# hzyu17/GaussianVI

Measured on AMD Instinct MI355X. Metric: sigma-point psi-evals/sec + NGD iters/sec, 1024-factor d=12 p=5 chain, higher is better.
Workload: dtype f64; 1 GPU; c3: T=1025 states, n=6; 1 step = 1 device-resident NGD iteration; restart every 30; factor_sets_columns=[K factors, d, GH degree p, N sigma points], factor_set_kinds=1024 x quadratic-prior d=12 p=5 (N=17217); 1025 x fixed-prior d=6 p=5 (N=1433), kernel_variant=6, chunks_per_factor=4, fused_pass=True, one_launch_factor_stage=False, mirror_pairs=False, fuse_trial=2

## Files before the change

gaussianvi_amd/_lib.py:

```python
from __future__ import annotations

import ctypes as C
import os

HERE = os.path.dirname(os.path.abspath(__file__))
LIB_PATH = os.environ.get("GVI_LIB_PATH") or os.path.join(HERE, "libgvi_hip.so")

c_double_p = C.POINTER(C.c_double)
c_int32_p = C.POINTER(C.c_int32)
c_int8_p = C.POINTER(C.c_int8)
c_void_pp = C.POINTER(C.c_void_p)
ALLGATHER_FN = C.CFUNCTYPE(C.c_int, C.c_void_p, C.c_void_p, C.c_void_p, C.c_int64, C.c_void_p)

SIGNATURES = {
    "gvi_ctx_create": [C.c_int, C.c_int, c_void_pp],
    "gvi_ctx_destroy": [C.c_void_p],
    "gvi_ctx_set_stream": [C.c_void_p, C.c_void_p],
    "gvi_ctx_sync": [C.c_void_p],
    "gvi_spgh_count": [C.c_int, C.c_int, C.POINTER(C.c_int64)],
    "gvi_spgh_nodes": [C.c_int, C.c_int, C.c_int64, C.c_void_p, C.c_void_p, C.c_void_p],
    "gvi_chain_set": [C.c_void_p, C.c_int, C.c_int],
    "gvi_factors_add": [C.c_void_p, C.c_int, C.c_int, C.c_int, C.c_void_p, C.c_int, C.c_void_p, C.c_int64,
                        C.c_void_p, C.POINTER(C.c_int)],
    "gvi_factors_add_table": [C.c_void_p, C.c_int, C.c_int, C.c_int, C.c_void_p, C.c_int, C.c_void_p, C.c_int64,
                              C.c_void_p, C.c_int64, C.c_void_p, C.c_void_p, C.POINTER(C.c_int)],
    "gvi_debug_cost_log": [C.c_void_p, C.c_int, C.c_void_p, C.POINTER(C.c_double)],
    "gvi_debug_asm_launches": [C.POINTER(C.c_int64), C.POINTER(C.c_int64)],
    "gvi_debug_fused_launches": [C.POINTER(C.c_int64)],
    "gvi_debug_block3_launches": [C.POINTER(C.c_int64)],
    "gvi_debug_products": [C.c_void_p, C.c_int, C.c_void_p, C.c_void_p, C.c_void_p, C.c_void_p, C.c_void_p],
    "gvi_factors_set_table": [C.c_void_p, C.c_int, C.c_int64, C.c_void_p, C.c_void_p],
    "gvi_factors_set_sdf2d": [C.c_void_p, C.c_int, C.c_double, C.c_double, C.c_double, C.c_int, C.c_int, C.c_void_p],
    "gvi_table_file_list": [C.c_char_p, C.c_int64, C.c_void_p, C.c_void_p, C.c_void_p, C.c_void_p],
    "gvi_table_file_read": [C.c_char_p, C.c_int, C.c_int, C.c_void_p, C.c_void_p, C.c_void_p],
    "gvi_table_file_write": [C.c_char_p, C.c_int, C.c_void_p, C.c_void_p],
    "gvi_ngd_trial_publish": [C.c_void_p],
    "gvi_ngd_trial_wait": [C.c_void_p, C.c_void_p],
    "gvi_ngd_spec_gradients_local": [C.c_void_p],
    "gvi_ngd_spec_gradients_finish": [C.c_void_p],
    "gvi_ngd_accept_spec": [C.c_void_p],
    "gvi_ngd_set_update_rule": [C.c_void_p, C.c_int],
    "gvi_prox_gradients": [C.c_void_p, C.c_double],
    "gvi_prox_trial": [C.c_void_p, C.c_double, C.c_void_p],
    "gvi_prox_step": [C.c_void_p, C.c_double, C.c_int, C.c_void_p, C.c_void_p, C.c_void_p, C.c_void_p],
    "gvi_factors_set_closed_form": [C.c_void_p, C.c_int, C.c_int],
    "gvi_factors_set_sdf3d": [C.c_void_p, C.c_int, C.c_void_p, C.c_double, C.c_int, C.c_int, C.c_int, C.c_void_p],
    "gvi_factors_set_arm": [C.c_void_p, C.c_int, C.c_int, C.c_void_p, C.c_void_p, C.c_void_p, C.c_void_p, C.c_int, C.c_void_p,
                            C.c_void_p, C.c_void_p],
    "gvi_factors_set_temperature": [C.c_void_p, C.c_int, C.c_void_p],
    "gvi_factors_set_params": [C.c_void_p, C.c_int, C.c_void_p, C.c_int64],
    "gvi_factors_set_readout_rule": [C.c_void_p, C.c_int, C.c_int],
    "gvi_factors_readout_info": [C.c_void_p, C.c_int, C.POINTER(C.c_int), C.POINTER(C.c_int), C.POINTER(C.c_int),
                                 C.POINTER(C.c_int64)],
    "gvi_factors_info": [C.c_void_p, C.c_int, C.POINTER(C.c_int), C.POINTER(C.c_int), C.POINTER(C.c_int),
                         C.POINTER(C.c_int64)],
    "gvi_moments": [C.c_void_p, C.c_int] + [C.c_void_p] * 5,
    "gvi_moments_dev": [C.c_void_p, C.c_int] + [C.c_void_p] * 5,
    "gvi_raw_moments": [C.c_void_p, C.c_int] + [C.c_void_p] * 5,
    "gvi_costs": [C.c_void_p, C.c_int] + [C.c_void_p] * 3,
    "gvi_costs_dev": [C.c_void_p, C.c_int] + [C.c_void_p] * 3,
    "gvi_expand": [C.c_void_p, C.c_int] + [C.c_void_p] * 3,
    "gvi_moments_from_psi": [C.c_void_p, C.c_int] + [C.c_void_p] * 6,
    "gvi_bt_assemble": [C.c_void_p, C.c_int, C.c_void_p, C.c_void_p, C.c_void_p, C.c_void_p, C.c_void_p, C.c_void_p],
# ... 96 lines not shown
```

gaussianvi_amd/api.py:

```python
from __future__ import annotations

import ctypes as C

import numpy as np

from . import _lib

PSI_RANGE_1D, PSI_QUAD_PRIOR, PSI_FIXED_PRIOR, PSI_HOST_CALLBACK, PSI_HINGE_SDF_2D = 0, 1, 2, 3, 4
PSI_HINGE_SDF_2D_BODY, PSI_HINGE_SDF_3D, PSI_HINGE_SDF_3D_ARM = 5, 6, 7
PSI_HINGE_SDF_2D_SEG, PSI_HINGE_SDF_3D_SEG = 8, 9
PSI_HINGE_BOX = 10
PSI_HINGE_HALFSPACE = 11
PSI_HINGE_BALLS_2D, PSI_HINGE_BALLS_3D = 13, 14
RULE_NGD, RULE_PROX_JKO = 0, 1
GVI_F64, GVI_F32 = 0, 1


class GviError(RuntimeError):
    def __init__(self, status, msg):
        super().__init__(f"gvi status {status}: {msg}")
        self.status = status


def _f64(a):
# ... 554 lines not shown
    def dist_init_callback(self, rank, world, fn):
        def trampoline(user, send, recv, count, stream):
            try:
                fn(send, recv, int(count), stream)
                return 0
            except Exception:
                import traceback
                traceback.print_exc()
                return 1
        self._allgather_cb = _lib.ALLGATHER_FN(trampoline)
        self._ck(self.lib.gvi_dist_init_callback(self.h, int(rank), int(world), C.cast(self._allgather_cb, C.c_void_p), None))

    def dist_info(self):
        r, w, n = C.c_int(), C.c_int(), C.c_int()
        self._ck(self.lib.gvi_dist_info(self.h, C.byref(r), C.byref(w), C.byref(n)))
        return dict(rank=r.value, world=w.value, records_per_rank=n.value)

    def debug_cost_log(self, entries=0, read=False):
        seq = C.c_double()
        if read:
            buf = np.zeros(self._dbg_entries)
            self._ck(self.lib.gvi_debug_cost_log(self.h, 0, _p(buf), C.byref(seq)))
            return buf, seq.value
        self._dbg_entries = entries if entries > 0 else 0
        self._ck(self.lib.gvi_debug_cost_log(self.h, entries if entries > 0 else -1, None, C.byref(seq)))
        return seq.value

    def debug_products(self, sid, K, d, m):
        S, Sinv, Lam = (np.zeros((K, d, d)) for _ in range(3))
        H, u0 = np.zeros((K, d, m)), np.zeros((K, m))
        self._ck(self.lib.gvi_debug_products(self.h, sid, _p(S), _p(Sinv), _p(Lam), _p(H) if m else None, _p(u0) if m else None))
        return dict(S=S, Sinv=Sinv, Lam=Lam, H=H, u0=u0)

    def set_variant(self, v):
        self._ck(self.lib.gvi_set_variant(self.h, v))

    def set_option(self, name, value):
        self._ck(self.lib.gvi_set_option(self.h, name.encode(), int(value)))


def context_for_chain(chain, device=0, specs=None, tables=None):
    ctx = Context(device)
    ctx.chain_set(chain["T"], chain["n"])
    ids = []
    if tables:
        ctx.set_option("trust_table_degree", 1)
    for spec in (chain["specs"] if specs is None else specs):
        ids.append(ctx.factors_add(spec["d"], spec["p"], spec["start"], spec["kind"], spec["params"],
                                   spec["temperature"], table=(tables or {}).get((spec["d"], spec["p"]))))
        if spec["kind"] in (PSI_HINGE_SDF_2D, PSI_HINGE_SDF_2D_BODY, PSI_HINGE_SDF_2D_SEG):
            ctx.factors_set_sdf2d(ids[-1], spec["sdf_origin"], spec["sdf_cell"], spec["sdf_field"])
        if spec["kind"] in (PSI_HINGE_SDF_3D, PSI_HINGE_SDF_3D_ARM, PSI_HINGE_SDF_3D_SEG):
            ctx.factors_set_sdf3d(ids[-1], spec["sdf_origin"], spec["sdf_cell"], spec["sdf_field"])
        if spec["kind"] == PSI_HINGE_SDF_3D_ARM:
            ctx.factors_set_arm(ids[-1], spec["arm"])
        if spec.get("readout_order"):
            ctx.factors_set_readout_rule(ids[-1], spec["readout_order"])
    return ctx, ids
```

gaussianvi_amd/csrc/api_inspect.inc:

```

gvi_status gvi_ngd_counters(gvi_ctx* ctx, int64_t* full_passes, int64_t* cost_passes, int reset) {
  if (!ctx) return GVI_ERR_ARG;
  if (full_passes) *full_passes = ctx->ngd.n_full_pass;
  if (cost_passes) *cost_passes = ctx->ngd.n_cost_pass;
  if (reset) ctx->ngd.n_full_pass = ctx->ngd.n_cost_pass = 0;
  return GVI_OK;
}

gvi_status gvi_debug_asm_launches(int64_t* dense, int64_t* generic) {
  if (dense) *dense = chain_asm_launches()[0].load();
  if (generic) *generic = chain_asm_launches()[1].load();
  return GVI_OK;
}

gvi_status gvi_debug_fused_launches(int64_t counts[3]) {
  if (!counts) return fail(nullptr, GVI_ERR_ARG, "NULL");
  for (int i = 0; i < 3; ++i) counts[i] = fused_launches()[i].load();
  return GVI_OK;
}

gvi_status gvi_debug_block3_launches(int64_t* count) {
  if (!count) return fail(nullptr, GVI_ERR_ARG, "NULL");
  *count = block3_launches().load();
  return GVI_OK;
// ... 131 lines not shown
    HIPCK(ctx, hipMemcpyToSymbol(HIP_SYMBOL(gvi_dbg_log), &lg, sizeof(double*)));
  } else if (entries == 0 && out) {
    if (!ctx->dbg_mask) return fail(ctx, GVI_ERR_STATE, "cost log not enabled");
    HIPCK(ctx, hipMemcpy(out, ctx->dbg_log.p, (size_t)(ctx->dbg_mask + 1) * 8, hipMemcpyDeviceToHost));
  } else {
    ctx->dbg_mask = 0;
    double* lg = nullptr;
    HIPCK(ctx, hipMemcpyToSymbol(HIP_SYMBOL(gvi_dbg_log), &lg, sizeof(double*)));
  }
  if (seq_now) *seq_now = ctx->seq;
  return GVI_OK;
}

gvi_status gvi_debug_products(gvi_ctx* ctx, int set_id, double* S, double* Sinv, double* Lam, double* H, double* u0) {
  if (!ctx) return GVI_ERR_ARG;
  FactorSet* s = get_set(ctx, set_id);
  if (!s) return GVI_ERR_ARG;
  HIPCK(ctx, hipSetDevice(ctx->device));
  GVICK(sync(ctx));
  const size_t dd = (size_t)s->K * s->d * s->d * 8, md = (size_t)s->K * s->m * s->d * 8, mb = (size_t)s->K * s->m * 8;
  auto get = [&](double* out, const DevMem& src, size_t bytes) {
    if (!out || bytes == 0) return hipSuccess;
    if (!src.p || src.bytes < bytes) return hipErrorInvalidValue;
    return hipMemcpy(out, src.p, bytes, hipMemcpyDeviceToHost);
  };
  HIPCK(ctx, get(S, s->S, dd));
  HIPCK(ctx, get(Sinv, s->Sinv, dd));
  HIPCK(ctx, get(Lam, s->Lam, dd));
  HIPCK(ctx, get(H, s->H, md));
  HIPCK(ctx, get(u0, s->u0, mb));
  return GVI_OK;
}

gvi_status gvi_set_variant(gvi_ctx* ctx, int variant) {
  return ctx && route_force_of_variant(variant, &ctx->force) ? GVI_OK : GVI_ERR_ARG;
}
```

gaussianvi_amd/csrc/dpp_rowb.hpp:

```cpp
#pragma once
#include <hip/hip_runtime.h>

namespace gvi {

template <int P, int WS>
__device__ __forceinline__ double rowb_mov(const double v) {
  double o;
  if constexpr (WS > 1) asm volatile("s_nop 4\n\tv_mov_b64_dpp %0, %1 row_newbcast:%2 row_mask:0xf bank_mask:0xf" : "=v"(o) : "v"(v), "n"(P));
  else asm volatile("s_nop 1\n\tv_mov_b64_dpp %0, %1 row_newbcast:%2 row_mask:0xf bank_mask:0xf" : "=v"(o) : "v"(v), "n"(P));
  return o;
}
template <int P>
__device__ __forceinline__ void rowb_fmac(double& c, const double b) {
  asm volatile("v_fmac_f64_dpp %0, %0, %1 row_newbcast:%2 row_mask:0xf bank_mask:0xf" : "+v"(c) : "v"(b), "n"(P));
}
template <int P>
__device__ __forceinline__ void rowb_fma(double& acc, const double src, const double mul) {
  asm volatile("v_fmac_f64_dpp %0, %1, -%2 row_newbcast:%3 row_mask:0xf bank_mask:0xf" : "+v"(acc) : "v"(src), "v"(mul), "n"(P));
}
__device__ __forceinline__ void rowb_pin(double& v) { asm volatile("" : "+v"(v)); }
__device__ __forceinline__ void rowb_settle(double& v) { asm volatile("s_nop 1" : "+v"(v)); }
template <int P>
__device__ __forceinline__ int rowb_int(const int v) { return __builtin_amdgcn_update_dpp(0, v, 0x150 + P, 0xf, 0xf, false); }

}
```

gaussianvi_amd/csrc/fused_timing.inc:

```

void fused_timing_dump(gvi_ctx* c, const FusedArgs& A, const unsigned long long* stamps) {
  unsigned long long h[1120];
  (void)hipStreamSynchronize(c->stream);
  (void)hipMemcpy(h, stamps, sizeof(h), hipMemcpyDeviceToHost);
  for (int blk = 0; blk < 8; ++blk)
    for (int w = 0; w < 4; ++w)
      for (int it = 0; it < 2; ++it) {
        const unsigned long long* ws = h + 352 + ((blk * 4 + w) * 2 + it) * 12;
        fprintf(stderr, "[walk stamps] block %4d wave %d item %d: shader cycles prologue %llu | s=1 %llu (%llu tiles) | s=2 %llu (%llu) | s=3 %llu (%llu) | s=4 %llu (%llu) | reduction %llu\n",
                blk * 146, w, it, ws[0], ws[1], ws[7], ws[2], ws[8], ws[3], ws[9], ws[4], ws[10], ws[5]);
      }
  for (int w = 0; w < 4; ++w) {
    fprintf(stderr, "[prep stamps] block 0 wave %d, us after the wave's start: prologue [arguments warm | first scalars | barrier] %.2f %.2f %.2f; gather [entry | loads back | stores issued] %.2f %.2f %.2f; products [Sigma row loaded | Cholesky | L^-1 | LDS | Lam + stores | H, u0]:",
            w, (double)(long long)(h[256 + 16 * w + 11] - h[8 * w]) * 0.01, (double)(long long)(h[256 + 16 * w + 12] - h[8 * w]) * 0.01,
            (double)(long long)(h[256 + 16 * w + 13] - h[8 * w]) * 0.01, (double)(long long)(h[256 + 16 * w + 8] - h[8 * w]) * 0.01, (double)(long long)(h[256 + 16 * w + 9] - h[8 * w]) * 0.01, (double)(long long)(h[256 + 16 * w + 10] - h[8 * w]) * 0.01);
    for (int i = 0; i < 6; ++i) fprintf(stderr, " %.2f", (double)(long long)(h[256 + 16 * w + i] - h[8 * w]) * 0.01);
    fprintf(stderr, "\n");
  }
  unsigned long long t0 = ~0ull;
  for (int blk = 0; blk < 8; ++blk) if (h[blk * 32] && h[blk * 32] < t0) t0 = h[blk * 32];
  for (int blk = 0; blk < 8; ++blk)
    for (int w = 0; w < 4; ++w) {
      const unsigned hw = (unsigned)h[320 + blk * 4 + w], xcc = (unsigned)(h[320 + blk * 4 + w] >> 32);
      fprintf(stderr, "[fused stamps] block %4d wave %d (xcc %u se %u cu %2u simd %u slot %2u; absolute, us after the first start):", blk * 146, w,
// ... 11 lines not shown
    const unsigned long long* q = hb.data() + (size_t)b * 5;
    if (!q[0] || !q[2]) continue;
    const unsigned hw = (unsigned)q[3], xcc = (unsigned)(q[3] >> 32) & 15;
    auto us = [&](unsigned long long t) { return (double)(long long)(t - tb0) * 0.01; };
    cus[(xcc << 8) | ((hw >> 8) & 255)].push_back({b, us(q[0]), us(q[1]), us(q[2]), us(q[4]), hw & 15});
  }
  std::vector<double> spread_bar, spread_end, first_bar, last_bar, walk_first, walk_last;
  int shown = 0;
  for (auto& [id, v] : cus) {
    std::sort(v.begin(), v.end(), [](const Blk& a, const Blk& b) { return a.bar < b.bar; });
    double e0 = 1e300, e1 = -1e300;
    for (const Blk& x : v) { e0 = std::min(e0, x.end); e1 = std::max(e1, x.end); }
    if (v.size() == 4) {
      spread_bar.push_back(v.back().bar - v.front().bar); spread_end.push_back(e1 - e0);
      first_bar.push_back(v.front().bar); last_bar.push_back(v.back().bar);
      walk_first.push_back(v.front().bar - v.front().start); walk_last.push_back(v.back().bar - v.back().start);
    }
    if (shown++ < 6)
      for (const Blk& x : v)
        fprintf(stderr, "[cu stamps] xcc %u se %u cu %2u: block %4d slot %2u, us after the first walk start: walk start %.2f, wave 0 ends phase 2 %.2f, "
                "behind the barrier %.2f, last exit %.2f\n", id >> 8, (id >> 5) & 7, id & 31, x.b, x.slot, x.start, x.p2, x.bar, x.end);
  }
  auto stat = [](std::vector<double> v, double* med, double* mx) {
    std::sort(v.begin(), v.end());
    *med = v.empty() ? 0.0 : v[v.size() / 2]; *mx = v.empty() ? 0.0 : v.back();
  };
  double m[6], x[6];
  stat(spread_bar, &m[0], &x[0]); stat(spread_end, &m[1], &x[1]); stat(first_bar, &m[2], &x[2]); stat(last_bar, &m[3], &x[3]);
  stat(walk_first, &m[4], &x[4]); stat(walk_last, &m[5], &x[5]);
  fprintf(stderr, "[cu summary] walk_prio %d, %zu CUs with four stamped blocks (of %zu): end of phase 2 (behind the barrier), first-to-last block of a CU: "
          "median %.2f max %.2f us; first block at median %.2f, last at median %.2f max %.2f us; walk (start to barrier) of the first block median %.2f, "
          "of the last median %.2f max %.2f us; last exit, first-to-last: median %.2f max %.2f us\n", A.walk_prio, spread_bar.size(), cus.size(),
          m[0], x[0], m[2], m[3], x[3], m[4], m[5], x[5], m[1], x[1]);
}
```

gaussianvi_amd/csrc/kernels_epilogue.hpp:

```cpp
#pragma once
#include <hip/hip_runtime.h>
#include <stdint.h>

#include "device_common.hpp"
#include "factor_dev.hpp"
#include "factor_lds.hpp"

namespace gvi {

struct EpiArgs {
  FactorDev f;
  const double* partial;
  int nchunk, full;
  double* Ephi;
  double* cost;
  double* Vdmu;
  double* Vddmu;
  double* E_xmuphi;
  double* E_xxphi;
};

template <int DT>
__device__ __forceinline__ double epilogue_body_t(const EpiArgs& a, int k, double* sm, int phase, const double* P, double* Zs = nullptr) {
  const FactorDev& f = a.f;
  const int d = DT ? DT : f.d, dd = d * d, lane = threadIdx.x & 63;
  const int npo = a.full ? npairs(d) : 1;
  const EpilogueLds L{d};
  double* Ms = sm + L.Ms();
  double* M2 = Ms + (L.M2() - L.Ms());
  double* Tm = M2 + (L.Tm() - L.M2());
  double* Sv = Zs ? Zs : Tm + (L.Sv() - L.Tm());
  double* Lv = Tm + (L.Lv() - L.Tm());
  const double Tk = f.temperature[k];
  const bool want_v = a.full && (a.Vdmu || a.Vddmu);
  if (want_v && phase != 2 && !Zs) {
    const double* Sinv = f.Sinv + (size_t)k * dd;
    const double* Lam = f.Lam + (size_t)k * dd;
    for (int e = lane; e < dd; e += 64) { Sv[e] = Sinv[e]; Lv[e] = Lam[e]; }
  }
  for (int j = lane; j < npo && phase != 2; j += 64) {
    double s = 0.0;
    for (int c0 = 0; c0 < a.nchunk; c0 += 8) {
      double pv[8];
#pragma unroll
      for (int q = 0; q < 8; ++q) pv[q] = c0 + q < a.nchunk ? P[(size_t)(c0 + q) * npo + j] : 0.0;
#pragma unroll
      for (int q = 0; q < 8; ++q) s += pv[q];
    }
    Ms[j] = s;
  }
  wave_lds_sync();
  const double m0 = Ms[0];
  const double costk = m0 / Tk;
  if (lane == 0 && phase != 2) {
    if (a.Ephi) a.Ephi[k] = m0;
    if (a.cost) a.cost[k] = costk;
  }
  if (!a.full || phase == 1) return costk;
  for (int e = lane; e < dd; e += 64) {
    const int i = e / d, j = e % d;
    M2[e] = i <= j ? Ms[pair_index(d, i, j)] : Ms[pair_index(d, j, i)];
  }
  wave_lds_sync();
  if (a.Vdmu) {
    for (int i = lane; i < d; i += 64) {
      double s = 0.0;
#pragma unroll
      for (int c = 0; c < d; ++c) s += Sv[i * d + c] * Ms[1 + c];
      a.Vdmu[(size_t)k * d + i] = s / Tk;
    }
  }
  if (a.Vddmu) {
    for (int e = lane; e < dd; e += 64) {
      const int i = e / d, j = e % d;
      double s = 0.0;
#pragma unroll
      for (int c = 0; c < d; ++c) s += Sv[i * d + c] * M2[c * d + j];
      Tm[e] = s;
    }
    wave_lds_sync();
    for (int e = lane; e < dd; e += 64) {
      const int i = e / d, j = e % d;
      if (i <= j) {
        double s = 0.0;
#pragma unroll
        for (int c = 0; c < d; ++c) s += Tm[i * d + c] * Sv[j * d + c];
        double lam;
        if (Zs) {
          lam = 0.0;
#pragma unroll
          for (int c = 0; c < d; ++c) lam = fma(Sv[i * d + c], Sv[j * d + c], lam);
        } else lam = Lv[i * d + j];
        const double v = (s - lam * m0) / Tk;
        a.Vddmu[(size_t)k * dd + i * d + j] = v;
        a.Vddmu[(size_t)k * dd + j * d + i] = v;
      }
    }
    wave_lds_sync();
  }
  if (a.E_xmuphi || a.E_xxphi) {
    const double* S = f.S + (size_t)k * dd;
    for (int e = lane; e < dd; e += 64) Sv[e] = S[e];
    wave_lds_sync();
  }
  if (a.E_xmuphi) {
    for (int i = lane; i < d; i += 64) {
      double s = 0.0;
#pragma unroll
      for (int c = 0; c < d; ++c) s += Sv[i * d + c] * Ms[1 + c];
      a.E_xmuphi[(size_t)k * d + i] = s;
    }
  }
  if (a.E_xxphi) {
    for (int e = lane; e < dd; e += 64) {
      const int i = e / d, j = e % d;
      double s = 0.0;
#pragma unroll
      for (int c = 0; c < d; ++c) s += Sv[i * d + c] * M2[c * d + j];
      Tm[e] = s;
    }
    wave_lds_sync();
    for (int e = lane; e < dd; e += 64) {
      const int i = e / d, j = e % d;
      double s = 0.0;
#pragma unroll
      for (int c = 0; c < d; ++c) s += Tm[i * d + c] * Sv[j * d + c];
      a.E_xxphi[(size_t)k * dd + e] = s;
    }
  }
  return costk;
}
// ... 69 lines not shown
    acc[0] = total;
    if (host_out) {
      publish_to_host(host_out, total + half_logdet[0], seq);
    }
  }
}

constexpr int EPI_GROUP = 64;
struct EpiTail {
  int on;
  double* acc;
  const double* half_logdet;
  double* host_out;
  double seq;
  unsigned* counter;
  const double* pred;
  double pred_val;
  double* accept;
  double* cost_dev;
  int slot_cur, slot_trial;
  int c0_use_imm;
  double c0_imm;
  int safe;
};

struct CostList {
  int nsets;
  double* cost[MAX_SETS];
  int K[MAX_SETS];
};

__device__ __forceinline__ void epi_tail_arrive(const CostList& cl, const EpiTail& tail, double* cost_slot, const double costk, const int lane,
                                                const unsigned bid, const unsigned nblocks, int* last) {
  if (lane == 0) {
    __hip_atomic_store(cost_slot, costk, __ATOMIC_RELAXED, __HIP_MEMORY_SCOPE_AGENT);
    asm volatile("s_waitcnt vmcnt(0)" ::: "memory");
    const unsigned grp = bid / EPI_GROUP, ngrp = (nblocks + EPI_GROUP - 1) / EPI_GROUP;
    const unsigned in_grp = grp + 1 < ngrp ? (unsigned)EPI_GROUP : nblocks - grp * EPI_GROUP;
    unsigned* gc = tail.counter + 32u * (1u + grp);
    int l = 0;
    const bool lastg = tail.safe ? __hip_atomic_fetch_add(gc, 1u, __ATOMIC_ACQ_REL, __HIP_MEMORY_SCOPE_AGENT) == in_grp - 1
                                 : __hip_atomic_fetch_add(gc, 1u, __ATOMIC_RELAXED, __HIP_MEMORY_SCOPE_AGENT) == in_grp - 1;
    if (lastg) {
      __hip_atomic_store(gc, 0u, __ATOMIC_RELAXED, __HIP_MEMORY_SCOPE_AGENT);
      l = ngrp == 1 ? 1
                    : (tail.safe ? __hip_atomic_fetch_add(tail.counter, 1u, __ATOMIC_ACQ_REL, __HIP_MEMORY_SCOPE_AGENT) == ngrp - 1
                                 : __hip_atomic_fetch_add(tail.counter, 1u, __ATOMIC_RELAXED, __HIP_MEMORY_SCOPE_AGENT) == ngrp - 1);
    }
    *last = l;
  }
  wave_lds_sync();
  if (!*last) return;
  double total = 0.0;
  for (int s2 = 0; s2 < cl.nsets; ++s2) {
    const double* cost = cl.cost[s2];
    const int K = cl.K[s2];
    double p[4][8];
#pragma unroll
    for (int j = 0; j < 4; ++j)
#pragma unroll
      for (int q = 0; q < 8; ++q) {
        const int k = lane + 64 * j + q * 256;
        p[j][q] = k < K ? __hip_atomic_load(cost + k, __ATOMIC_RELAXED, __HIP_MEMORY_SCOPE_AGENT) : 0.0;
      }
    double vs[4];
#pragma unroll
    for (int j = 0; j < 4; ++j) {
      double s = 0.0;
#pragma unroll
      for (int q = 0; q < 8; ++q) s += p[j][q];
      for (int k0 = lane + 64 * j + 8 * 256; k0 < K; k0 += 8 * 256) {
        double pp[8];
#pragma unroll
        for (int q = 0; q < 8; ++q) {
          const int k = k0 + q * 256;
          pp[q] = k < K ? __hip_atomic_load(cost + k, __ATOMIC_RELAXED, __HIP_MEMORY_SCOPE_AGENT) : 0.0;
        }
#pragma unroll
        for (int q = 0; q < 8; ++q) s += pp[q];
      }
      vs[j] = s;
    }
    double t = (vs[0] + vs[2]) + (vs[1] + vs[3]);
#pragma unroll
    for (int w = 32; w > 0; w >>= 1) t += __shfl_down(t, w);
    total += __shfl(t, 0);
  }
  if (lane == 0) {
    __hip_atomic_store(tail.counter, 0u, __ATOMIC_RELAXED, __HIP_MEMORY_SCOPE_AGENT);
    tail.acc[0] = total;
    const double c1 = total + tail.half_logdet[0];
    if (tail.host_out) publish_to_host(tail.host_out, c1, tail.seq);
    if (tail.accept) {
      const double c0 = tail.c0_use_imm ? tail.c0_imm : tail.cost_dev[tail.slot_cur];
      tail.cost_dev[tail.slot_trial] = c1;
      tail.accept[0] = c1 < c0 ? tail.seq : 0.0;
    }
  }
  wave_lds_sync();
}

__global__ __launch_bounds__(64) void epilogue_all_kernel(EpiList L, EpiTail tail, CostList cl) {
  extern __shared__ double sm[];
  if (pred_skip(tail.pred, tail.pred_val)) return;
  int si = 0;
  while (si + 1 < L.nsets && (int)blockIdx.x >= L.koff[si + 1]) ++si;
  const int kf = (int)blockIdx.x - L.koff[si];
  if (!tail.on) { epilogue_body(L.e[si], kf, sm); return; }
  const double costk = epilogue_body(L.e[si], kf, sm, 1);
  __shared__ int last;
  epi_tail_arrive(cl, tail, L.e[si].cost + kf, costk, (int)threadIdx.x, blockIdx.x, gridDim.x, &last);
  epilogue_body(L.e[si], kf, sm, 2);
}

__global__ __launch_bounds__(256) void expand_kernel(FactorDev f, const double* __restrict__ mu,
                                                     double* __restrict__ X) {
  const int k = blockIdx.y, d = f.d;
  const int64_t i = (int64_t)blockIdx.x * 256 + threadIdx.x;
  if (i >= f.N) return;
  const double* S = f.S + (size_t)k * d * d;
  for (int r = 0; r < d; ++r) {
    double x = mu[(size_t)k * d + r];
    for (int c = 0; c < d; ++c) x += S[r * d + c] * f.Zt[(size_t)c * f.Np + i];
    X[((size_t)k * d + r) * f.N + i] = x;
  }
}

}
```

gaussianvi_amd/csrc/kernels_fused.hpp:

```cpp
#pragma once
#include "device_common.hpp"
#include "factor_lds.hpp"
#include "kernels_epilogue.hpp"
#include "kernels_orbit.hpp"
#include "kernels_prep.hpp"

namespace gvi {

constexpr int FUSED_MAX_ITEMS = 4;
constexpr int FUSED_BLOCK_STAMPS = 1100;
#ifdef GVI_FUSED_TIMING
__device__ int gvi_fused_exp;
#endif

struct FusedSet {
  FactorDev f;
  OrbitArgs oa;
  const double* mu;
  const double* Sigma;
  const int32_t* start;
  double* mu_k;
  double* Sigma_k;
  double* Ephi;
  double* cost;
  double* Vdmu;
  double* Vddmu;
};

struct FusedArgs {
  int nsets;
  int nblk;
  int koff[3];
  FusedSet s[2];
  int gather, n;
  const double* gmu;
  const double* gdmu;
// ... 39 lines not shown
    else p = A.SigU + (size_t)s * nn + c * n + (r - n);
    v[i] = e < dd ? *p : 0.0;
  }
  double m = 0.0;
  if (lane < DT) {
    const size_t j = (size_t)s * n + lane;
    m = A.gdmu ? A.gmu[j] + A.gstep * A.gdmu[j] : A.gmu[j];
  }
#ifdef GVI_FUSED_TIMING
  asm volatile("s_waitcnt vmcnt(0) lgkmcnt(0)" ::: "memory");
#endif
  PREP_STAMP(9);
  if (pred_fail(lpred)) return true;
#pragma unroll
  for (int i = 0; i < NI; ++i) {
    const int e = lane + 64 * i;
    if (e < dd) { Sl[e] = v[i]; S.Sigma_k[(size_t)k * dd + e] = v[i]; }
  }
  if (lane < DT) { ml[lane] = m; S.mu_k[(size_t)k * DT + lane] = m; }
  PREP_STAMP(10);
  return false;
}

template <int M, int SMAX, int WAVES, int D0, int D1>
__global__ __launch_bounds__(256, WAVES) void factor_fused_kernel(FusedArgs A, int dmax, int copies_max, int maxitems, [[maybe_unused]] unsigned long long* stamps) {
  extern __shared__ double sm[];
#ifdef GVI_FUSED_TIMING
#define FUSED_STAMP(i) do { const unsigned long long t_ = (i) == 0 ? t_start : __builtin_amdgcn_s_memrealtime(); if (stamps && (threadIdx.x & 63) == 0 && (blockIdx.x % 146) == 0) stamps[(blockIdx.x / 146) * 32 + (threadIdx.x >> 6) * 8 + (i)] = t_; } while (0)
  const unsigned long long t_start = __builtin_amdgcn_s_memrealtime();
#else
#define FUSED_STAMP(i) do { } while (0)
#endif
#ifdef GVI_FUSED_TIMING
  if (blockIdx.x == 0 && threadIdx.x == 0) { gvi_prep_stamps = stamps ? stamps + 8 * 32 : nullptr; gvi_walk_stamps = stamps ? stamps + 352 : nullptr; }
  unsigned long long* const bstamps = stamps && blockIdx.x < FUSED_BLOCK_STAMPS ? stamps + 1120 + blockIdx.x * 5 : nullptr;
#define FUSED_BLOCK_STAMP(i) do { if (bstamps && threadIdx.x == 0) bstamps[i] = __builtin_amdgcn_s_memrealtime(); } while (0)
  struct ExitStamp {
    unsigned long long* p;
    __device__ ~ExitStamp() { if (p && (threadIdx.x & 63) == 0) atomicMax(p, (unsigned long long)__builtin_amdgcn_s_memrealtime()); }
  } exit_stamp{bstamps ? bstamps + 4 : nullptr};
  if (bstamps && threadIdx.x == 0)
    bstamps[3] = (unsigned long long)__builtin_amdgcn_s_getreg((31 << 11) | 4) | ((unsigned long long)__builtin_amdgcn_s_getreg((31 << 11) | 20) << 32);
#else
#define FUSED_BLOCK_STAMP(i) do { } while (0)
#endif
  FUSED_STAMP(0);
#ifdef GVI_FUSED_TIMING
  if (stamps && (threadIdx.x & 63) == 0 && (blockIdx.x % 146) == 0)
    stamps[320 + (blockIdx.x / 146) * 4 + (threadIdx.x >> 6)] = (unsigned long long)__builtin_amdgcn_s_getreg((31 << 11) | 4) |
                                                                   ((unsigned long long)__builtin_amdgcn_s_getreg((31 << 11) | 20) << 32);
#endif
  const double* const pred_p = A.tail.pred;
  const int nblk_ = A.nblk, K0 = A.s[0].f.K, K1_ = A.s[1].f.K, nsets_ = A.nsets;
  constexpr int KA_LINES = (sizeof(FusedArgs) + 3 * 8 + 63) / 64;
  static_assert(KA_LINES == 28, "kernarg_warm: one specialisation per argument block size");
  kernarg_warm<KA_LINES>();
  PREP_STAMP(11);
  asm volatile("" :: "s"(pred_p), "s"(nblk_), "s"(K0), "s"(K1_), "s"(nsets_));
  PREP_STAMP(12);
  const LazyPred lpred = pred_issue(pred_p, A.tail.pred_val);
  const int wave = __builtin_amdgcn_readfirstlane(threadIdx.x >> 6);
  const int b = (int)blockIdx.x;
  if (b >= nblk_) {
    const int64_t j = (int64_t)(b - A.nblk) * 256 + threadIdx.x;
    const double v = j < A.nmu ? A.gmu[j] + A.gstep * A.gdmu[j] : 0.0;
    if (pred_fail(lpred)) return;
    if (j < A.nmu) A.mu_out[j] = v;
// ... 112 lines not shown
  FUSED_BLOCK_STAMP(1);
  __syncthreads();
  FUSED_STAMP(4);
  FUSED_BLOCK_STAMP(2);
  const bool helpers = A.tail.on && nitems <= 2;
  if (iw >= nitems) {
    const int it = iw - 2;
    if (!helpers || it < 0 || it >= nitems) return;
    const int si = it < c0 ? 0 : 1;
    const int k = b + (it < c0 ? it : it - c0) * A.nblk;
    const FusedSet& S = A.s[si];
    const double Tk = S.f.temperature[k];
    const double* Pl = Pbase + (size_t)it * ps;
    const int npo = npairs(S.f.d);
    double m0 = 0.0;
#pragma unroll
    for (int q = 0; q < 4; ++q) m0 += Pl[(size_t)q * npo];
    const double costk = m0 / Tk;
    epi_tail_arrive(A.cl, A.tail, S.cost + k, costk, (int)(threadIdx.x & 63), (unsigned)(A.koff[si] + k), (unsigned)A.koff[A.nsets],
                    (int*)(sm + (size_t)wave * region));
    return;
  }
  {
    const int si = iw < c0 ? 0 : 1;
    const int k = b + (iw < c0 ? iw : iw - c0) * A.nblk;
    const FusedSet& S = A.s[si];
    const int d = S.f.d;
    double* area = sm + (size_t)wave * region;
    double* Zs = Zbase + (size_t)iw * zs;
    const double* Pl = Pbase + (size_t)iw * ps;
    EpiArgs e;
    e.f = S.f; e.partial = nullptr; e.nchunk = 4; e.full = 1;
    e.Ephi = S.Ephi; e.cost = helpers ? nullptr : S.cost; e.Vdmu = S.Vdmu; e.Vddmu = S.Vddmu; e.E_xmuphi = nullptr; e.E_xxphi = nullptr;
    auto epi = [&](int phase) { return si == 0 ? epilogue_body_t<D0>(e, k, area, phase, Pl, Zs) : epilogue_body_t<D1>(e, k, area, phase, Pl, Zs); };
    if (!A.tail.on || helpers) { epi(0); return; }
    const double costk = epi(1);
    FUSED_STAMP(5);
    int* last = (int*)(area + EpilogueLds{d}.last());
    epi_tail_arrive(A.cl, A.tail, S.cost + k, costk, (int)(threadIdx.x & 63), (unsigned)(A.koff[si] + k), (unsigned)A.koff[A.nsets], last);
    FUSED_STAMP(6);
    epi(2);
    FUSED_STAMP(7);
  }
}

}
```

gaussianvi_amd/csrc/launch_factor.inc:

```

namespace {

template <int D, int R>
gvi_status launch_split(gvi_ctx* c, const MomArgs& a, dim3 grid, hipStream_t st) {
  const size_t lds = (size_t)SPLIT_LDS_DOUBLES(D) * 8;
  GVICK(allow_lds(c, (const void*)moments_split_kernel<D, R, true>, (int)lds));
  GVICK(allow_lds(c, (const void*)moments_split_kernel<D, R, false>, (int)lds));
  if (a.full) hipLaunchKernelGGL((moments_split_kernel<D, R, true>), grid, dim3(256), lds, st, a);
  else hipLaunchKernelGGL((moments_split_kernel<D, R, false>), grid, dim3(256), lds, st, a);
  return GVI_OK;
}

template <int D, typename Psi>
void launch_reg(const MomArgs& a, dim3 grid, hipStream_t st) {
  if (a.full) hipLaunchKernelGGL((moments_reg_kernel<D, Psi, true>), grid, dim3(256), 0, st, a);
  else hipLaunchKernelGGL((moments_reg_kernel<D, Psi, false>), grid, dim3(256), 0, st, a);
}

template <int D, int M>
void launch_sreg(const MomArgs& a, dim3 grid, hipStream_t st, bool pipe) {
  if (a.full && pipe) hipLaunchKernelGGL((moments_sreg_kernel<D, M, true, true>), grid, dim3(256), 0, st, a);
  else if (a.full) hipLaunchKernelGGL((moments_sreg_kernel<D, M, true>), grid, dim3(256), 0, st, a);
  else hipLaunchKernelGGL((moments_sreg_kernel<D, M, false>), grid, dim3(256), 0, st, a);
}
// ... 96 lines not shown

inline std::atomic<long long>& block3_launches() { static std::atomic<long long> c; return c; }

gvi_status fused_round_blocks(gvi_ctx* c, const void* kernel, size_t lds, int* out) {
  const auto key = std::make_pair(kernel, lds);
  auto it = c->fused_round.find(key);
  if (it == c->fused_round.end()) {
    int per_cu = 0, cus = 0;
    HIPCK(c, hipOccupancyMaxActiveBlocksPerMultiprocessor(&per_cu, kernel, 256, lds));
    HIPCK(c, hipDeviceGetAttribute(&cus, hipDeviceAttributeMultiprocessorCount, c->device));
    it = c->fused_round.emplace(key, per_cu * cus).first;
  }
  *out = it->second;
  return GVI_OK;
}

#ifdef GVI_FUSED_TIMING
#include "fused_timing.inc"
#endif

template <int M, int SMAX, int WAVES, int D0, int D1>
gvi_status launch_fused_t(gvi_ctx* c, FusedArgs& A, unsigned grid, size_t lds, int dmax, int copies, int items, hipEvent_t e0, hipEvent_t e1) {
  const void* const kernel = (const void*)factor_fused_kernel<M, SMAX, WAVES, D0, D1>;
  if (lds > 64 * 1024) GVICK(allow_lds(c, kernel, (int)lds));
  if (A.walk_prio) {
    int round = 0;
    GVICK(fused_round_blocks(c, kernel, lds, &round));
    if (A.nblk > round) A.walk_prio = 0;
  }
#ifdef GVI_FUSED_TIMING
  const int dbg = getenv("GVI_FUSED_DBG") ? atoi(getenv("GVI_FUSED_DBG")) : 0;
  static unsigned long long* stamps = nullptr;
  static int nprint = 0;
  constexpr size_t nstamps = 1120 + 5 * FUSED_BLOCK_STAMPS;
  if ((dbg & 8) && !stamps) {
    if (hipMalloc(&stamps, nstamps * 8) != hipSuccess) stamps = nullptr; else (void)hipMemset(stamps, 0, nstamps * 8);
    const int exp = (dbg >> 4) & 7;
    (void)hipMemcpyToSymbol(HIP_SYMBOL(gvi_fused_exp), &exp, sizeof(exp));
  }
#else
  const int dbg = 0;
  unsigned long long* stamps = nullptr;
#endif
  hipExtLaunchKernelGGL((factor_fused_kernel<M, SMAX, WAVES, D0, D1>), dim3(grid), dim3(256), (uint32_t)lds, c->stream, e0, e1, 0, A, dmax, copies, items,
                        (dbg & 8) ? stamps : (unsigned long long*)nullptr);
  ++fused_launches()[M == 2 ? 2 : (SMAX <= 4 ? 0 : 1)];
#ifdef GVI_FUSED_TIMING
  if ((dbg & 8) && stamps && ++nprint > 200 && nprint <= 202) fused_timing_dump(c, A, stamps);
#endif
  return GVI_OK;
}

gvi_status launch_prep(gvi_ctx* c, const FactorDev& f, const double* mu, const double* Sigma, hipStream_t st) {
  const size_t lds = prep_lds_bytes(f.d);
  if (!with_prep_instance(f.d, [&]<int EPLP>(PrepInst<EPLP>) { hipLaunchKernelGGL(prep_kernel<EPLP>, dim3(f.K), dim3(64), lds, st, f, mu, Sigma); }))
    return fail(c, GVI_ERR_UNSUPPORTED, "factor dimension > 32");
  return GVI_OK;
}

gvi_status run_prep(gvi_ctx* c, FactorSet& s, const double* mu, const double* Sigma, int slot = -1,
                    hipStream_t st = nullptr) {
  if (!st) st = c->stream;
  if (slot >= 0 && s.prep_slot == slot) return GVI_OK;
  s.prep_slot = slot;
  if (s.K == 0) return GVI_OK;
  GVICK(launch_prep(c, s.dev(c->opt), mu, Sigma, st));
  HIPCK(c, hipGetLastError());
// ... 293 lines not shown
```

include/gvi_hip.h:

```cpp
#ifndef GVI_HIP_H
#define GVI_HIP_H

#include <stdint.h>

#ifdef __cplusplus
extern "C" {
#endif

typedef struct gvi_ctx gvi_ctx;
typedef int gvi_status;

enum {
  GVI_OK = 0,
  GVI_ERR_ARG = 1,
  GVI_ERR_HIP = 2,
  GVI_ERR_UNSUPPORTED = 3,
  GVI_ERR_NOTABLE = 4,
  GVI_ERR_STATE = 5
};
enum { GVI_F64 = 0, GVI_F32 = 1 };

enum { GVI_PSI_RANGE_1D = 0, GVI_PSI_QUAD_PRIOR = 1, GVI_PSI_FIXED_PRIOR = 2, GVI_PSI_HOST_CALLBACK = 3,
       GVI_PSI_HINGE_SDF_2D = 4, GVI_PSI_HINGE_SDF_2D_BODY = 5, GVI_PSI_HINGE_SDF_3D = 6, GVI_PSI_HINGE_SDF_3D_ARM = 7,
       GVI_PSI_HINGE_SDF_2D_SEG = 8, GVI_PSI_HINGE_SDF_3D_SEG = 9, GVI_PSI_HINGE_BOX = 10,
// ... 115 lines not shown
gvi_status gvi_ngd_cov_columns_dev(gvi_ctx* ctx, int ncols, const int32_t* nodes, double* C_dev);

gvi_status gvi_interp_set(gvi_ctx* ctx, int Q, const int32_t* idx, const double* A, const double* B, const double* c,
                          const double* Qt);
gvi_status gvi_interp_info(gvi_ctx* ctx, int* Q, int* nbad);
gvi_status gvi_bt_interp(gvi_ctx* ctx, const double* mu, const double* SigD, const double* SigU, double* mean_q, double* cov_q);
gvi_status gvi_ngd_interp(gvi_ctx* ctx, double* mean_q, double* cov_q);
gvi_status gvi_ngd_interp_dev(gvi_ctx* ctx, double* mean_q_dev, double* cov_q_dev);
gvi_status gvi_bt_interp_samples(gvi_ctx* ctx, int S, const double* X, uint64_t noise_seed, int64_t first, const double* eps,
                                 double* Xq);
gvi_status gvi_ngd_sample_interp(gvi_ctx* ctx, int S, uint64_t seed, uint64_t noise_seed, int64_t first, double* X, double* Xq);
gvi_status gvi_ngd_sample_interp_dev(gvi_ctx* ctx, int S, uint64_t seed, uint64_t noise_seed, int64_t first, double* X_dev,
                                     double* Xq_dev);

gvi_status gvi_sample_factor_costs(gvi_ctx* ctx, int set_id, int S, const double* X, double* cost);
gvi_status gvi_sample_clearance(gvi_ctx* ctx, int set_id, int S, const double* X, double* clr);
gvi_status gvi_sample_clearance_dev(gvi_ctx* ctx, int set_id, int S, const double* X_dev, double* clr_dev);
gvi_status gvi_sample_costs(gvi_ctx* ctx, int S, const double* X, double* J);
gvi_status gvi_sample_costs_dev(gvi_ctx* ctx, int S, const double* X_dev, double* J_dev);
gvi_status gvi_ngd_sample_costs(gvi_ctx* ctx, int S, uint64_t seed, int64_t first, int clearance_set, double* X, double* J,
                                double* logq, double* clr_min);
gvi_status gvi_ngd_sample_costs_dev(gvi_ctx* ctx, int S, uint64_t seed, int64_t first, int clearance_set, double* X_dev,
                                    double* J_dev, double* logq_dev, double* clr_min_dev);

gvi_status gvi_profile_enable(gvi_ctx* ctx, int on);
gvi_status gvi_profile_last(gvi_ctx* ctx, int set_id, int what , float* ms);
gvi_status gvi_profile_stages(gvi_ctx* ctx, int on, float* mean_us, int* counts);
gvi_status gvi_profile_geometry(gvi_ctx* ctx, int set_id, int* variant, int* nchunk, int64_t* chunk);
gvi_status gvi_debug_cost_log(gvi_ctx* ctx, int entries, double* out, double* seq_now);
gvi_status gvi_debug_asm_launches(int64_t* dense, int64_t* generic);
gvi_status gvi_debug_fused_launches(int64_t counts[3]);
gvi_status gvi_debug_block3_launches(int64_t* count);
gvi_status gvi_debug_products(gvi_ctx* ctx, int set_id, double* S, double* Sinv, double* Lam, double* H, double* u0);
gvi_status gvi_set_variant(gvi_ctx* ctx, int variant);
gvi_status gvi_set_option(gvi_ctx* ctx, const char* name, int value);

#ifdef __cplusplus
}
#endif
#endif
```

Before: 235.8 billion psi-evals/s.

## Compute fused epilogue Hessian products with DPP row-broadcast FMAs in registers

Replaces the fused kernel's LDS-based epilogue, which ran the two d×d matrix products per factor through shared-memory loops with lane-strided indexing, with a register version. Each 16-lane row holds one column of M2 plus the m1 column, and the products use DPP row-broadcast FMAs. Vdmu and Vddmu are written straight from registers. The goal is to cut LDS traffic, sync points and integer index math in the per-factor tail. The old path is kept behind timing build flags, and the change also adds epilogue timing stamps and a debug readback API for factor outputs.

New measurement: 235.5 billion psi-evals/s. About the same (-0.1%).

```diff
diff --git a/gaussianvi_amd/_lib.py b/gaussianvi_amd/_lib.py
--- a/gaussianvi_amd/_lib.py
+++ b/gaussianvi_amd/_lib.py
@@ -29,6 +29,7 @@
     "gvi_debug_fused_launches": [C.POINTER(C.c_int64)],
     "gvi_debug_block3_launches": [C.POINTER(C.c_int64)],
     "gvi_debug_products": [C.c_void_p, C.c_int, C.c_void_p, C.c_void_p, C.c_void_p, C.c_void_p, C.c_void_p],
+    "gvi_debug_factor_outputs": [C.c_void_p, C.c_int, C.c_void_p, C.c_void_p, C.c_void_p, C.c_void_p],
     "gvi_factors_set_table": [C.c_void_p, C.c_int, C.c_int64, C.c_void_p, C.c_void_p],
     "gvi_factors_set_sdf2d": [C.c_void_p, C.c_int, C.c_double, C.c_double, C.c_double, C.c_int, C.c_int, C.c_void_p],
     "gvi_table_file_list": [C.c_char_p, C.c_int64, C.c_void_p, C.c_void_p, C.c_void_p, C.c_void_p],
diff --git a/gaussianvi_amd/api.py b/gaussianvi_amd/api.py
--- a/gaussianvi_amd/api.py
+++ b/gaussianvi_amd/api.py
@@ -610,6 +610,11 @@
         self._ck(self.lib.gvi_debug_products(self.h, sid, _p(S), _p(Sinv), _p(Lam), _p(H) if m else None, _p(u0) if m else None))
         return dict(S=S, Sinv=Sinv, Lam=Lam, H=H, u0=u0)
 
+    def debug_factor_outputs(self, sid, K, d):
+        Ephi, cost, Vdmu, Vddmu = np.empty(K), np.empty(K), np.empty((K, d)), np.empty((K, d, d))
+        self._ck(self.lib.gvi_debug_factor_outputs(self.h, sid, _p(Ephi), _p(cost), _p(Vdmu), _p(Vddmu)))
+        return Ephi, cost, Vdmu, Vddmu
+
     def set_variant(self, v):
         self._ck(self.lib.gvi_set_variant(self.h, v))
 
diff --git a/gaussianvi_amd/csrc/api_inspect.inc b/gaussianvi_amd/csrc/api_inspect.inc
--- a/gaussianvi_amd/csrc/api_inspect.inc
+++ b/gaussianvi_amd/csrc/api_inspect.inc
@@ -187,6 +187,25 @@
   return GVI_OK;
 }
 
+gvi_status gvi_debug_factor_outputs(gvi_ctx* ctx, int set_id, double* Ephi, double* cost, double* Vdmu, double* Vddmu) {
+  if (!ctx) return GVI_ERR_ARG;
+  FactorSet* s = get_set(ctx, set_id);
+  if (!s) return GVI_ERR_ARG;
+  HIPCK(ctx, hipSetDevice(ctx->device));
+  GVICK(sync(ctx));
+  const size_t K = (size_t)s->K, d = (size_t)s->d;
+  auto get = [&](double* out, const DevMem& src, size_t bytes) {
+    if (!out || bytes == 0) return hipSuccess;
+    if (!src.p || src.bytes < bytes) return hipErrorInvalidValue;
+    return hipMemcpy(out, src.p, bytes, hipMemcpyDeviceToHost);
+  };
+  HIPCK(ctx, get(Ephi, s->Ephi, K * 8));
+  HIPCK(ctx, get(cost, s->cost, K * 8));
+  HIPCK(ctx, get(Vdmu, s->Vdmu, K * d * 8));
+  HIPCK(ctx, get(Vddmu, s->Vddmu, K * d * d * 8));
+  return GVI_OK;
+}
+
 gvi_status gvi_set_variant(gvi_ctx* ctx, int variant) {
   return ctx && route_force_of_variant(variant, &ctx->force) ? GVI_OK : GVI_ERR_ARG;
 }
diff --git a/gaussianvi_amd/csrc/dpp_rowb.hpp b/gaussianvi_amd/csrc/dpp_rowb.hpp
--- a/gaussianvi_amd/csrc/dpp_rowb.hpp
+++ b/gaussianvi_amd/csrc/dpp_rowb.hpp
@@ -20,6 +20,7 @@
 }
 __device__ __forceinline__ void rowb_pin(double& v) { asm volatile("" : "+v"(v)); }
 __device__ __forceinline__ void rowb_settle(double& v) { asm volatile("s_nop 1" : "+v"(v)); }
+__device__ __forceinline__ void rowb_converged() { asm volatile("s_nop 4" ::: "memory"); }
 template <int P>
 __device__ __forceinline__ int rowb_int(const int v) { return __builtin_amdgcn_update_dpp(0, v, 0x150 + P, 0xf, 0xf, false); }
 
diff --git a/gaussianvi_amd/csrc/fused_timing.inc b/gaussianvi_amd/csrc/fused_timing.inc
--- a/gaussianvi_amd/csrc/fused_timing.inc
+++ b/gaussianvi_amd/csrc/fused_timing.inc
@@ -67,4 +67,26 @@
           "median %.2f max %.2f us; first block at median %.2f, last at median %.2f max %.2f us; walk (start to barrier) of the first block median %.2f, "
           "of the last median %.2f max %.2f us; last exit, first-to-last: median %.2f max %.2f us\n", A.walk_prio, spread_bar.size(), cus.size(),
           m[0], x[0], m[2], m[3], x[3], m[4], m[5], x[5], m[1], x[1]);
+  unsigned long long he[EPI_STAMP_WORDS];
+  (void)hipMemcpy(he, stamps + 1120 + 5 * (size_t)FUSED_BLOCK_STAMPS, sizeof(he), hipMemcpyDeviceToHost);
+  for (int blk = 0; blk < 8; ++blk)
+    for (int w = 0; w < 4; ++w) {
+      const unsigned long long* q = he + blk * 32 + w * 8;
+      const unsigned long long bar = hb[(size_t)blk * 146 * 5 + 2];
+      if (!q[0] || !q[4] || !bar) continue;
+      auto us = [&](unsigned long long t) { return (double)(long long)(t - bar) * 0.01; };
+      fprintf(stderr, "[epi stamps] block %4d wave %d, us behind the block's phase-2 barrier: entry %.2f | chunk sums, cost out %.2f | first product %.2f | "
+              "second product %.2f | last store issued %.2f\n", blk * 146, w, us(q[0]), us(q[1]), us(q[2]), q[3] ? us(q[3]) : -1.0, us(q[4]));
+    }
+  const unsigned long long* tl = he + 8 * 32;
+  if (tl[3]) {
+    unsigned long long end = 0;
+    for (int b = 0; b < A.nblk && b < FUSED_BLOCK_STAMPS; ++b) end = std::max(end, hb[(size_t)b * 5 + 4]);
+    const int lb = (int)tl[4];
+    const unsigned long long bar = lb < FUSED_BLOCK_STAMPS ? hb[(size_t)lb * 5 + 2] : 0;
+    auto rel = [&](unsigned long long t, unsigned long long ref) { return ref ? (double)(long long)(t - ref) * 0.01 : -1.0; };
+    fprintf(stderr, "[tail stamps] last arriver block %d, us behind its phase-2 barrier: entry %.2f | arrival counted %.2f | costs summed %.2f | published %.2f; "
+            "the publish is %.2f us after the first walk start and %.2f us before the latest exit of any block\n", lb, rel(tl[0], bar), rel(tl[1], bar),
+            rel(tl[2], bar), rel(tl[3], bar), rel(tl[3], tb0), rel(end, tl[3]));
+  }
 }
diff --git a/gaussianvi_amd/csrc/kernels_epilogue.hpp b/gaussianvi_amd/csrc/kernels_epilogue.hpp
--- a/gaussianvi_amd/csrc/kernels_epilogue.hpp
+++ b/gaussianvi_amd/csrc/kernels_epilogue.hpp
@@ -19,6 +19,32 @@
   double* E_xmuphi;
   double* E_xxphi;
 };
+
+constexpr int EPI_STAMP_WORDS = 8 * 32 + 8;
+#ifdef GVI_FUSED_TIMING
+__device__ unsigned long long* gvi_epi_stamps;
+#define EPI_STAMP(on, i) do { const unsigned long long t_ = __builtin_amdgcn_s_memrealtime(); if ((on) && (blockIdx.x % 146) == 0 && blockIdx.x / 146 < 8 && (threadIdx.x & 63) == 0 && gvi_epi_stamps) gvi_epi_stamps[(blockIdx.x / 146) * 32 + (threadIdx.x >> 6) * 8 + (i)] = t_; } while (0)
+#define EPI_TAIL_STAMP(i, v) do { if (gvi_epi_stamps) gvi_epi_stamps[8 * 32 + (i)] = (v); } while (0)
+#else
+#define EPI_STAMP(on, i) do { } while (0)
+#define EPI_TAIL_STAMP(i, v) do { } while (0)
+#endif
+
+__device__ __forceinline__ double epi_chunk_sum(const double* P, const int nchunk, const int npo, const int j) {
+  double s = 0.0;
+  for (int c0 = 0; c0 < nchunk; c0 += 8) {
+    double pv[8];
+#pragma unroll
+    for (int q = 0; q < 8; ++q) pv[q] = c0 + q < nchunk ? P[(size_t)(c0 + q) * npo + j] : 0.0;
+#pragma unroll
+    for (int q = 0; q < 8; ++q) s += pv[q];
+  }
+  return s;
+}
+__device__ __forceinline__ double epi_close_num(const double s, const double lam, const double m0) { return s - lam * m0; }
+__device__ __forceinline__ double epi_close(const double s, const double lam, const double m0, const double Tk) {
+  return epi_close_num(s, lam, m0) / Tk;
+}
 
 template <int DT>
 __device__ __forceinline__ double epilogue_body_t(const EpiArgs& a, int k, double* sm, int phase, const double* P, double* Zs = nullptr) {
@@ -38,16 +64,9 @@
     const double* Lam = f.Lam + (size_t)k * dd;
     for (int e = lane; e < dd; e += 64) { Sv[e] = Sinv[e]; Lv[e] = Lam[e]; }
   }
+  if (phase != 2) EPI_STAMP(Zs != nullptr, 0);
   for (int j = lane; j < npo && phase != 2; j += 64) {
-    double s = 0.0;
-    for (int c0 = 0; c0 < a.nchunk; c0 += 8) {
-      double pv[8];
-#pragma unroll
-      for (int q = 0; q < 8; ++q) pv[q] = c0 + q < a.nchunk ? P[(size_t)(c0 + q) * npo + j] : 0.0;
-#pragma unroll
-      for (int q = 0; q < 8; ++q) s += pv[q];
-    }
-    Ms[j] = s;
+    Ms[j] = epi_chunk_sum(P, a.nchunk, npo, j);
   }
   wave_lds_sync();
   const double m0 = Ms[0];
@@ -56,6 +75,7 @@
     if (a.Ephi) a.Ephi[k] = m0;
     if (a.cost) a.cost[k] = costk;
   }
+  if (phase != 2) EPI_STAMP(Zs != nullptr, 1);
   if (!a.full || phase == 1) return costk;
   for (int e = lane; e < dd; e += 64) {
     const int i = e / d, j = e % d;
@@ -79,6 +99,7 @@
       Tm[e] = s;
     }
     wave_lds_sync();
+    EPI_STAMP(Zs != nullptr, 2);
     for (int e = lane; e < dd; e += 64) {
       const int i = e / d, j = e % d;
       if (i <= j) {
@@ -91,12 +112,13 @@
 #pragma unroll
           for (int c = 0; c < d; ++c) lam = fma(Sv[i * d + c], Sv[j * d + c], lam);
         } else lam = Lv[i * d + j];
-        const double v = (s - lam * m0) / Tk;
+        const double v = epi_close(s, lam, m0, Tk);
         a.Vddmu[(size_t)k * dd + i * d + j] = v;
         a.Vddmu[(size_t)k * dd + j * d + i] = v;
       }
     }
     wave_lds_sync();
+    EPI_STAMP(Zs != nullptr, 4);
   }
   if (a.E_xmuphi || a.E_xxphi) {
     const double* S = f.S + (size_t)k * dd;
@@ -232,6 +254,9 @@
 
 __device__ __forceinline__ void epi_tail_arrive(const CostList& cl, const EpiTail& tail, double* cost_slot, const double costk, const int lane,
                                                 const unsigned bid, const unsigned nblocks, int* last) {
+#ifdef GVI_FUSED_TIMING
+  const unsigned long long t_entry = __builtin_amdgcn_s_memrealtime();
+#endif
   if (lane == 0) {
     __hip_atomic_store(cost_slot, costk, __ATOMIC_RELAXED, __HIP_MEMORY_SCOPE_AGENT);
     asm volatile("s_waitcnt vmcnt(0)" ::: "memory");
@@ -251,6 +276,9 @@
   }
   wave_lds_sync();
   if (!*last) return;
+#ifdef GVI_FUSED_TIMING
+  const unsigned long long t_counted = __builtin_amdgcn_s_memrealtime();
+#endif
   double total = 0.0;
   for (int s2 = 0; s2 < cl.nsets; ++s2) {
     const double* cost = cl.cost[s2];
@@ -286,6 +314,9 @@
     for (int w = 32; w > 0; w >>= 1) t += __shfl_down(t, w);
     total += __shfl(t, 0);
   }
+#ifdef GVI_FUSED_TIMING
+  const unsigned long long t_summed = __builtin_amdgcn_s_memrealtime();
+#endif
   if (lane == 0) {
     __hip_atomic_store(tail.counter, 0u, __ATOMIC_RELAXED, __HIP_MEMORY_SCOPE_AGENT);
     tail.acc[0] = total;
@@ -296,6 +327,11 @@
       tail.cost_dev[tail.slot_trial] = c1;
       tail.accept[0] = c1 < c0 ? tail.seq : 0.0;
     }
+#ifdef GVI_FUSED_TIMING
+    asm volatile("s_waitcnt vmcnt(0)" ::: "memory");
+    EPI_TAIL_STAMP(0, t_entry); EPI_TAIL_STAMP(1, t_counted); EPI_TAIL_STAMP(2, t_summed);
+    EPI_TAIL_STAMP(3, (unsigned long long)__builtin_amdgcn_s_memrealtime()); EPI_TAIL_STAMP(4, (unsigned long long)blockIdx.x);
+#endif
   }
   wave_lds_sync();
 }
diff --git a/gaussianvi_amd/csrc/kernels_epilogue_rowb.hpp b/gaussianvi_amd/csrc/kernels_epilogue_rowb.hpp
--- /dev/null
+++ b/gaussianvi_amd/csrc/kernels_epilogue_rowb.hpp
@@ -0,0 +1,99 @@
+#pragma once
+#include "dpp_rowb.hpp"
+#include "kernels_epilogue.hpp"
+
+namespace gvi {
+
+__host__ __device__ constexpr int epi_rowb_base(const int d, const int a) { return 1 + d + a * d - a * (a - 1) / 2 - a; }
+constexpr bool epi_rowb_index_ok() {
+  for (int d = 1; d <= 15; ++d)
+    for (int a = 0; a < d; ++a) {
+      if (epi_rowb_base(d, a) < 1 + a) return false;
+      for (int b = a; b < d; ++b) {
+        const int right = epi_rowb_base(d, a) + b, wrong = epi_rowb_base(d, b) + a;
+        if (right != 1 + d + a * d - a * (a - 1) / 2 + (b - a) || right > wrong) return false;
+      }
+    }
+  return true;
+}
+static_assert(epi_rowb_index_ok(), "epilogue_rowb_t: the packed index of M2[c'][c] as a minimum");
+
+template <int DT, int R, int C>
+__device__ __forceinline__ void epi_rowb_first(double (&t1)[R], double (&lam)[R], const double (&wcol)[R], const double (&nm2)[DT],
+                                               const double (&nwrow)[DT]) {
+  if constexpr (C < DT) {
+#pragma unroll
+    for (int r = 0; r < R; ++r) rowb_fma<C>(t1[r], wcol[r], nm2[C]);
+#pragma unroll
+    for (int r = 0; r < R; ++r) rowb_fma<C>(lam[r], wcol[r], nwrow[C]);
+    epi_rowb_first<DT, R, C + 1>(t1, lam, wcol, nm2, nwrow);
+  }
+}
+template <int DT, int R, int C>
+__device__ __forceinline__ void epi_rowb_second(double (&t2)[R], const double (&t1)[R], const double (&nwrow)[DT]) {
+  if constexpr (C < DT) {
+#pragma unroll
+    for (int r = 0; r < R; ++r) rowb_fma<C>(t2[r], t1[r], nwrow[C]);
+    epi_rowb_second<DT, R, C + 1>(t2, t1, nwrow);
+  }
+}
+
+template <int DT>
+__device__ __forceinline__ double epilogue_rowb_t(const EpiArgs& a, const int k, double* sm, const int phase, const double* P, const double* Zs) {
+  static_assert(DT >= 1 && DT <= 15, "one 16-lane row holds the d columns of M2 and m1 behind them");
+  constexpr int d = DT, dd = DT * DT, R = (DT + 3) / 4, npo = npairs(DT);
+  const int lane = (int)__builtin_amdgcn_mbcnt_hi(~0u, __builtin_amdgcn_mbcnt_lo(~0u, 0u)), q = lane >> 4, c = lane & 15;
+  double* Ms = sm + EpilogueLds{d}.Ms();
+  const double Tk = a.f.temperature[k];
+  if (phase != 2) EPI_STAMP(true, 0);
+  for (int j = lane; j < npo && phase != 2; j += 64) Ms[j] = epi_chunk_sum(P, a.nchunk, npo, j);
+  wave_lds_sync();
+  const double m0 = Ms[0];
+  const double costk = m0 / Tk;
+  if (lane == 0 && phase != 2) {
+    if (a.Ephi) a.Ephi[k] = m0;
+    if (a.cost) a.cost[k] = costk;
+  }
+  if (phase != 2) EPI_STAMP(true, 1);
+  if (phase == 1 || !(a.Vdmu || a.Vddmu)) return costk;
+  const int cr = c < d ? c : 0;
+  double wcol[R], nwrow[DT], nm2[DT];
+#pragma unroll
+  for (int r = 0; r < R; ++r) {
+    const int i = q * R + r;
+    const bool in = i < d && c < d;
+    const double w = Zs[in ? i * d + c : 0];
+    wcol[r] = in ? w : 0.0;
+  }
+#pragma unroll
+  for (int cc = 0; cc < d; ++cc) nwrow[cc] = -Zs[cr * d + cc];
+  const int rb = c < d ? epi_rowb_base(d, cr) : 1;
+#pragma unroll
+  for (int cc = 0; cc < d; ++cc) nm2[cc] = -Ms[min(epi_rowb_base(d, cc) + cr, rb + cc)];
+  double t1[R], t2[R], lam[R];
+#pragma unroll
+  for (int r = 0; r < R; ++r) { t1[r] = 0.0; t2[r] = 0.0; lam[r] = 0.0; }
+  rowb_converged();
+#pragma unroll
+  for (int r = 0; r < R; ++r) rowb_settle(wcol[r]);
+  epi_rowb_first<DT, R, 0>(t1, lam, wcol, nm2, nwrow);
+  EPI_STAMP(true, 2);
+#pragma unroll
+  for (int r = 0; r < R; ++r) rowb_settle(t1[r]);
+  epi_rowb_second<DT, R, 0>(t2, t1, nwrow);
+  EPI_STAMP(true, 3);
+#pragma unroll
+  for (int r = 0; r < R; ++r) {
+    const int i = q * R + r;
+    const double v = (c == d ? t1[r] : epi_close_num(t2[r], lam[r], m0)) / Tk;
+    if (i < d && c == d && a.Vdmu) a.Vdmu[(size_t)k * d + i] = v;
+    if (i < d && c < d && i <= c && a.Vddmu) {
+      a.Vddmu[(size_t)k * dd + i * d + c] = v;
+      a.Vddmu[(size_t)k * dd + c * d + i] = v;
+    }
+  }
+  EPI_STAMP(true, 4);
+  return costk;
+}
+
+}
diff --git a/gaussianvi_amd/csrc/kernels_fused.hpp b/gaussianvi_amd/csrc/kernels_fused.hpp
--- a/gaussianvi_amd/csrc/kernels_fused.hpp
+++ b/gaussianvi_amd/csrc/kernels_fused.hpp
@@ -2,6 +2,7 @@
 #include "device_common.hpp"
 #include "factor_lds.hpp"
 #include "kernels_epilogue.hpp"
+#include "kernels_epilogue_rowb.hpp"
 #include "kernels_orbit.hpp"
 #include "kernels_prep.hpp"
 
@@ -107,7 +108,7 @@
 #define FUSED_STAMP(i) do { } while (0)
 #endif
 #ifdef GVI_FUSED_TIMING
-  if (blockIdx.x == 0 && threadIdx.x == 0) { gvi_prep_stamps = stamps ? stamps + 8 * 32 : nullptr; gvi_walk_stamps = stamps ? stamps + 352 : nullptr; }
+  if (blockIdx.x == 0 && threadIdx.x == 0) { gvi_prep_stamps = stamps ? stamps + 8 * 32 : nullptr; gvi_walk_stamps = stamps ? stamps + 352 : nullptr; gvi_epi_stamps = stamps ? stamps + 1120 + 5 * FUSED_BLOCK_STAMPS : nullptr; }
   unsigned long long* const bstamps = stamps && blockIdx.x < FUSED_BLOCK_STAMPS ? stamps + 1120 + blockIdx.x * 5 : nullptr;
 #define FUSED_BLOCK_STAMP(i) do { if (bstamps && threadIdx.x == 0) bstamps[i] = __builtin_amdgcn_s_memrealtime(); } while (0)
   struct ExitStamp {
@@ -286,7 +287,11 @@
     EpiArgs e;
     e.f = S.f; e.partial = nullptr; e.nchunk = 4; e.full = 1;
     e.Ephi = S.Ephi; e.cost = helpers ? nullptr : S.cost; e.Vdmu = S.Vdmu; e.Vddmu = S.Vddmu; e.E_xmuphi = nullptr; e.E_xxphi = nullptr;
+#if defined(GVI_FUSED_TIMING) && defined(GVI_FUSED_EPI_LDS)
     auto epi = [&](int phase) { return si == 0 ? epilogue_body_t<D0>(e, k, area, phase, Pl, Zs) : epilogue_body_t<D1>(e, k, area, phase, Pl, Zs); };
+#else
+    auto epi = [&](int phase) { return si == 0 ? epilogue_rowb_t<D0>(e, k, area, phase, Pl, Zs) : epilogue_rowb_t<D1>(e, k, area, phase, Pl, Zs); };
+#endif
     if (!A.tail.on || helpers) { epi(0); return; }
     const double costk = epi(1);
     FUSED_STAMP(5);
diff --git a/gaussianvi_amd/csrc/launch_factor.inc b/gaussianvi_amd/csrc/launch_factor.inc
--- a/gaussianvi_amd/csrc/launch_factor.inc
+++ b/gaussianvi_amd/csrc/launch_factor.inc
@@ -152,7 +152,7 @@
   const int dbg = getenv("GVI_FUSED_DBG") ? atoi(getenv("GVI_FUSED_DBG")) : 0;
   static unsigned long long* stamps = nullptr;
   static int nprint = 0;
-  constexpr size_t nstamps = 1120 + 5 * FUSED_BLOCK_STAMPS;
+  constexpr size_t nstamps = 1120 + 5 * FUSED_BLOCK_STAMPS + EPI_STAMP_WORDS;
   if ((dbg & 8) && !stamps) {
     if (hipMalloc(&stamps, nstamps * 8) != hipSuccess) stamps = nullptr; else (void)hipMemset(stamps, 0, nstamps * 8);
     const int exp = (dbg >> 4) & 7;
diff --git a/include/gvi_hip.h b/include/gvi_hip.h
--- a/include/gvi_hip.h
+++ b/include/gvi_hip.h
@@ -171,6 +171,7 @@
 gvi_status gvi_debug_fused_launches(int64_t counts[3]);
 gvi_status gvi_debug_block3_launches(int64_t* count);
 gvi_status gvi_debug_products(gvi_ctx* ctx, int set_id, double* S, double* Sinv, double* Lam, double* H, double* u0);
+gvi_status gvi_debug_factor_outputs(gvi_ctx* ctx, int set_id, double* Ephi, double* cost, double* Vdmu, double* Vddmu);
 gvi_status gvi_set_variant(gvi_ctx* ctx, int variant);
 gvi_status gvi_set_option(gvi_ctx* ctx, const char* name, int value);
 
```
